# jerry102102102/RL_brain_trainer

Hardware: AMD Instinct MI355X
Metric: env-steps/sec (whole node), Stage-5 Approach->Finisher PPO loops (rollout + update); value = the Approach loop, finisher.value = the Finisher loop (higher is better)
Workload: dtype f32

## Files before the change

### include/kp1_ppo.h

```cpp
#ifndef KP1_PPO_H
#define KP1_PPO_H

#include <stdint.h>

#include "kp1.h"

#ifdef __cplusplus
extern "C" {
#endif

int kp1_gae_scan(int32_t device, const float* rewards, const float* values, const uint8_t* dones, const float* last_values,
                 float gamma, float gae_lambda, float* advantages, float* returns, int32_t T, int32_t N, void* stream);

int kp1_gae_scan_replicas(int32_t device, const float* rewards, const float* values, const uint8_t* dones, const float* last_values,
                          const float* gamma_lambda, int32_t n_per_replica, float* advantages, float* returns, int32_t T, int32_t N, void* stream);

int kp1_bootstrap_truncated(int32_t device, float* rewards, const float* terminal_values, const uint8_t* dones, float gamma,
                            int64_t count, void* stream);

int kp1_adv_minibatch_sums(int32_t device, const float* advantages, const int64_t* idx, int64_t total, int64_t minibatch, double* out_sums,
                           void* stream);
int kp1_random_permutation(int32_t device, int64_t n, const uint32_t* keys, int64_t* out, void* stream);

int kp1_adv_minibatch_stats(int32_t device, const double* sums, int64_t n_minibatches, float* out_stats, void* stream);
// ... 102 lines not shown
                             float* log_prob, float* next_obs, float* reward, uint8_t* done, float* terminal_obs, void* stream);

int kp1_eval_step(kp1_mlp* m, kp1_env* env, float* obs, float* reward, uint8_t* done, const kp1_eval_buffers* buffers, int32_t step,
                  const double* ready_thresholds , int32_t confirm_steps, void* stream);

int kp1_mlp_loss_grad(kp1_mlp* m, const float* obs, int32_t obs_stride, const int64_t* idx, int32_t n, const float* actions,
                      const float* old_log_prob, const float* advantages, const float* returns, float adv_mean, float adv_inv_std,
                      const float* adv_stats_dev, float clip_range, float ent_coef, float vf_coef, float inv_count, float* grad_out,
                      float* stats_out, int32_t grad_is_zero, void* stream);

#define KP1_MLP_OPT_FUSED 1
#define KP1_MLP_OPT_ACTOR_EXTRA_STEPS 2
#define KP1_MLP_OPT_STEP_COUNT 3
#define KP1_MLP_OPT_PROFILE 4
#define KP1_MLP_OPT_BF16X3_WGRAD 5
#define KP1_MLP_PROFILE_SLOTS 4
#define KP1_MLP_PROFILE_TILE 0
#define KP1_MLP_PROFILE_WGRAD 1
#define KP1_MLP_PROFILE_FINALIZE 2
#define KP1_MLP_PROFILE_ADAM 3
int kp1_mlp_set_option(kp1_mlp* m, int32_t option, int32_t value);
int kp1_mlp_profile_read(kp1_mlp* m, float* out_us , int32_t* out_launches );

int kp1_mlp_adam_step(kp1_mlp* m, float* params, float* grad, float* exp_avg, float* exp_avg_sq, float lr, float eps,
                      float max_grad_norm, int32_t step, int32_t flags, void* stream);

int kp1_mlp_anchor_loss_grad(kp1_mlp* m, const float* obs, int32_t obs_stride, const int64_t* idx, int32_t n, const float* teacher_actions,
                             float loss_weight, float* grad_out, float* loss_out, void* stream);

int kp1_mlp_anchor_adam_step(kp1_mlp* m, float* params, float* grad, float* exp_avg, float* exp_avg_sq, float lr, float eps,
                             float max_grad_norm, int32_t step, void* stream);

int kp1_mlp_placement_check(int32_t device, int32_t n_rows, int32_t* out, void* stream);
int kp1_mlp_time_kernels(kp1_mlp* m, const float* obs, int32_t obs_stride, int32_t n, int32_t iters, float* out_ms, double* out_flops,
                         void* stream);

int kp1_set_obs_stride(kp1_env* env, int32_t stride);

#ifdef __cplusplus
}
#endif
#endif
```

### rl_brain_trainer_amd/csrc/kp1_mlp.hip

```cpp
#include <hip/hip_runtime.h>
#include <hip/hip_ext.h>

#include <cmath>
#include <cstddef>
#include <cstdlib>
#include <cstring>
#include <vector>

#include "../../include/kp1_ppo.h"
#include "kp1_device.hpp"
#include "kp1_host.hpp"

using kp1::fail;
using namespace kp1;

typedef float f32x16 __attribute__((ext_vector_type(16)));
typedef float f32x4 __attribute__((ext_vector_type(4)));

namespace {

constexpr int ACT = KP1_MLP_ACT, HEADS = 8;
constexpr float LOG_SQRT_2PI = 0.9189385332046727f;

enum { EPI_BIAS_TANH = 0, EPI_DTANH = 1 };
// ... 818 lines not shown
  } else if (i < L.a_w) {
    r.p = a.hpart + 9 * Hp + (i - L.v_b2);
  } else if (i < L.a_b) {
    const int64_t e = i - L.a_w;
    r.p = a.hpart + (e / H) * Hp + e % H;
  } else if (i < L.c_w) {
    r.p = a.hpart + 10 * Hp + (i - L.a_b);
  } else if (i < L.c_b) {
    r.p = a.hpart + 7 * Hp + (i - L.c_w);
  } else {
    r.p = a.hpart + 10 * Hp + 7;
  }
  return r;
}

__host__ __device__ inline int64_t finalize_wide_count(const ParamLayout& L) { return ACT + 4 * (int64_t)L.H + (L.total - L.a_w); }
__device__ __forceinline__ int64_t finalize_wide_index(const ParamLayout& L, int64_t e) {
  const int H = L.H;
  if (e < ACT) return L.log_std + e;
  e -= ACT;
  if (e < H) return L.p_b1 + e;
  e -= H;
  if (e < H) return L.p_b2 + e;
  e -= H;
  if (e < H) return L.v_b1 + e;
  e -= H;
  if (e < H) return L.v_b2 + e;
  e -= H;
  return L.a_w + e;
}

__host__ __device__ inline int64_t finalize_vec_items(const ParamLayout& L) { return 2 * ((int64_t)L.H * L.H / 4 + (int64_t)L.H * L.IN / 4); }

template <bool POP = false>
__global__ void __launch_bounds__(256) grad_finalize_kernel(const FinalizeArgs a_, int n_main) {
  const FinalizeArgs a = POP ? finalize_args_replica(a_, blockIdx.y) : a_;
  const ParamLayout& L = a.L;
  __shared__ double sq[4];
  __shared__ float red[8][32];
  float gval = 0.f;
  double gsq = 0.0;
  if ((int)blockIdx.x < n_main) {
    const int64_t j = (int64_t)(blockIdx.x * 256u + threadIdx.x);
    const int64_t per2 = (int64_t)L.H * L.H / 4, per1 = (int64_t)L.H * L.IN / 4;
    if (j < 2 * (per2 + per1)) {
      const float* src;
      int64_t stride, dst;
      int n;
      if (j < 2 * per2) {
        const int net = j >= per2;
        const unsigned rem = (unsigned)(j - net * per2), q4 = (unsigned)(L.H / 4), row = rem / q4, c4 = rem - row * q4;
        src = a.slab2 + net * a.s2_net + (int64_t)row * a.s2_ld + 4 * c4;
        stride = a.s2_chunk; n = a.s2_n;
        dst = (net ? L.v_w2 : L.p_w2) + (int64_t)row * L.H + 4 * c4;
      } else {
        const int64_t k = j - 2 * per2;
        const int net = k >= per1;
        const unsigned rem = (unsigned)(k - net * per1), q4 = (unsigned)(L.IN / 4), row = rem / q4, c4 = rem - row * q4;
        src = a.slab1 + net * a.s1_net + (int64_t)row * a.s1_ld + 4 * c4;
        stride = a.s1_chunk; n = a.s1_n;
        dst = (net ? L.v_w1 : L.p_w1) + (int64_t)row * L.IN + 4 * c4;
      }
      f32x4 s = {0.f, 0.f, 0.f, 0.f};
      int c = 0;
      for (; c + 32 <= n; c += 32) {
        f32x4 v[32];
#pragma unroll
        for (int u = 0; u < 32; ++u) v[u] = *reinterpret_cast<const f32x4*>(src + (int64_t)(c + u) * stride);
#pragma unroll
        for (int u = 0; u < 32; ++u) s += v[u];
      }
      for (; c + 16 <= n; c += 16) {
        f32x4 v[16];
#pragma unroll
        for (int u = 0; u < 16; ++u) v[u] = *reinterpret_cast<const f32x4*>(src + (int64_t)(c + u) * stride);
#pragma unroll
        for (int u = 0; u < 16; ++u) s += v[u];
      }
      for (; c + 8 <= n; c += 8) {
        f32x4 v[8];
#pragma unroll
        for (int u = 0; u < 8; ++u) v[u] = *reinterpret_cast<const f32x4*>(src + (int64_t)(c + u) * stride);
#pragma unroll
        for (int u = 0; u < 8; ++u) s += v[u];
      }
      for (; c < n; ++c) s += *reinterpret_cast<const f32x4*>(src + (int64_t)c * stride);
#pragma unroll
      for (int q = 0; q < 4; ++q) {
        a.grad[dst + q] = s[q];
        gsq += (double)s[q] * (double)s[q];
      }
    }
    if (a.step_counter && blockIdx.x == 0 && threadIdx.x == 0) *a.step_counter += 1;
    if (a.stats && blockIdx.x == 0 && threadIdx.x == 3) {
      float ent = 0.f;
      for (int k = 0; k < ACT; ++k) ent += 0.5f + LOG_SQRT_2PI + a.log_std[k];
      a.stats[2] += ent;
    }
  } else {
    const int64_t n_wide = finalize_wide_count(L);
    const int el = threadIdx.x & 31, strand = threadIdx.x >> 5;
    const int64_t e = (int64_t)(blockIdx.x - n_main) * 32 + el;
    const bool is_grad = e < n_wide, is_stat = !is_grad && e < n_wide + 3;
    PartialSrc s{};
    int64_t flat = 0;
    if (is_grad) {
      flat = finalize_wide_index(L, e);
      s = finalize_source(a, flat);
    } else if (is_stat) {
      s.p = a.hpart + 10 * L.Hp + 15 + (e - n_wide);
      s.stride = a.h_stride; s.n = a.h_n; s.add = 0.f;
    }
    float part = 0.f;
    if (is_grad || is_stat) {
      int c = strand;
      for (; c + 8 * 31 < s.n; c += 8 * 32) {
        float v[32];
#pragma unroll
        for (int u = 0; u < 32; ++u) v[u] = s.p[(int64_t)(c + 8 * u) * s.stride];
#pragma unroll
        for (int u = 0; u < 32; ++u) part += v[u];
      }
      for (; c < s.n; c += 8) part += s.p[(int64_t)c * s.stride];
    }
    red[strand][el] = part;
    __syncthreads();
    if (threadIdx.x < 32) {
      float t = red[0][el];
#pragma unroll
      for (int k = 1; k < 8; ++k) t += red[k][el];
      if (is_grad) {
        gval = t + s.add;
        a.grad[flat] = gval;
      } else if (is_stat && a.stats) {
        const int k = (int)(e - n_wide);
        a.stats[k == 2 ? 3 : k] += t * a.inv_count;
      }
    }
  }
  double w = gsq + (double)gval * (double)gval;
  for (int off = 32; off > 0; off >>= 1) w += __shfl_xor(w, off);
  if ((threadIdx.x & 63) == 0) sq[threadIdx.x >> 6] = w;
  __syncthreads();
  if (threadIdx.x == 0) a.sumsq[blockIdx.x] = ((sq[0] + sq[1]) + sq[2]) + sq[3];
}

template <bool POP = false>
__global__ void __launch_bounds__(256) sumsq_partials_kernel(const float* __restrict__ g, int64_t n, double* __restrict__ partials, unsigned r_partials) {
  __shared__ double s[256];
  if constexpr (POP) {
    g += blockIdx.y * (unsigned)n;
    partials += blockIdx.y * r_partials;
  }
  double a = 0.0;
  for (int64_t i = (int64_t)blockIdx.x * 256 + threadIdx.x; i < n; i += (int64_t)gridDim.x * 256) a += (double)g[i] * (double)g[i];
  s[threadIdx.x] = a;
  __syncthreads();
  for (int k = 128; k > 0; k >>= 1) {
    if (threadIdx.x < k) s[threadIdx.x] += s[threadIdx.x + k];
    __syncthreads();
  }
  if (threadIdx.x == 0) partials[blockIdx.x] = s[0];
}

constexpr int ADAM_BLOCK = 256, VEC = 1;
template <bool POP = false>
__global__ void __launch_bounds__(ADAM_BLOCK) adam_kernel(float* __restrict__ p, float* __restrict__ g, float* __restrict__ m, float* __restrict__ v,
                                                   int64_t n, const double* __restrict__ partials, int n_partials, float lr, float eps, float max_norm,
                                                   float bc1, float bc2_sqrt, const ParamLayout L, const Packed k_, int zero_grad,
                                                   const int* __restrict__ step_counter, int host_step, const int* __restrict__ actor_extra,
                                                   unsigned r_partials, const float* __restrict__ hparams) {
// ... 253 lines not shown
    m[i] = mn; v[i] = vn; p[i] = pn;
    pack_one(i, pn, L, k);
  }
}

__global__ void anchor_count_kernel(int* __restrict__ actor_extra) { *actor_extra += 1; }

#include "kp1_env_step.inc"
#include "kp1_eval_step.inc"
#include "kp1_mlp_tile.inc"
#include "kp1_mlp_fused.inc"

}

struct kp1_mlp {
  int device = 0, H = 0, Hp = 0, max_batch = 0;
  int K = 1;
  ParamLayout L;
  Packed k{};
  float* h1 = nullptr;
  float* h2 = nullptr;
  float* dz2 = nullptr;
  float* dz1 = nullptr;
  float* xf = nullptr;
  int bf16x3 = 0;
  unsigned short* sp_h1 = nullptr; unsigned short* sp_dz2 = nullptr; unsigned short* sp_dz1 = nullptr; unsigned short* sp_xf = nullptr;
  double* partials = nullptr;
  double* anchor_partials = nullptr;
  float* slab = nullptr;
  float* slab1 = nullptr;
  float* bslab = nullptr;
  float* hpart = nullptr;
  int n_finalize_blocks = 0;
  int* step_dev = nullptr;
  float* hparams_dev = nullptr;
  bool hparams_on = false;
  int last_s2_n = 0, last_s1_n = 0;
  int fused = 1;
  const float* last_params = nullptr;
  bool slab_stale = false;
  std::vector<void*> allocs;
  int profile = 0;
  struct ProfPair { hipEvent_t a, b; };
  std::vector<ProfPair> prof[KP1_MLP_PROFILE_SLOTS];
  int prof_used[KP1_MLP_PROFILE_SLOTS] = {0, 0, 0, 0};
};

namespace {
struct ProfSlotInFlight { hipEvent_t a = nullptr, b = nullptr; bool attached = false; };
thread_local ProfSlotInFlight tl_prof;

struct ProfScope {
  kp1_mlp* m; int slot; hipStream_t stream; bool on;
  ProfScope(kp1_mlp* m_, int slot_, hipStream_t s_) : m(m_), slot(slot_), stream(s_), on(m_->profile != 0) {
    if (!on) return;
    auto& v = m->prof[slot];
    if (m->prof_used[slot] >= (int)v.size()) {
      kp1_mlp::ProfPair p{};
      if (hipEventCreate(&p.a) != hipSuccess || hipEventCreate(&p.b) != hipSuccess) { on = false; return; }
      v.push_back(p);
    }
    tl_prof.a = v[m->prof_used[slot]].a;
    tl_prof.b = v[m->prof_used[slot]].b;
    tl_prof.attached = false;
  }
  ~ProfScope() {
    if (!on) return;
    if (!tl_prof.attached) {
      (void)hipEventRecord(tl_prof.a, stream);
      (void)hipEventRecord(tl_prof.b, stream);
    }
    tl_prof = ProfSlotInFlight{};
    m->prof_used[slot] += 1;
  }
};

#define KP1_LAUNCH(kernel, grid, block, bytes, stream, ...)                                                        \
  do {                                                                                                             \
    if (tl_prof.a != nullptr && !tl_prof.attached) {                                                               \
      tl_prof.attached = true;                                                                                     \
      hipExtLaunchKernelGGL(kernel, grid, block, bytes, stream, tl_prof.a, tl_prof.b, 0, __VA_ARGS__);             \
    } else {                                                                                                       \
      hipLaunchKernelGGL(kernel, grid, block, bytes, stream, __VA_ARGS__);                                         \
    }                                                                                                              \
  } while (0)
}

namespace {

constexpr int N_PARTIALS = 128;
constexpr int ANCHOR_PARTIALS = 256;
constexpr int PARTIALS_STRIDE = 2 * N_PARTIALS + 2048;
constexpr int TN_SPLIT2 = 8, TN_SPLIT1 = 16;

int tn_chunk_rows(int n, int tiles) {
  int chunks = (256 + tiles - 1) / tiles;
  if (chunks > 64) chunks = 64;
  if (chunks < 1) chunks = 1;
  int rows = (n + chunks - 1) / chunks;
  rows = (rows + 63) / 64 * 64;
  return rows < 64 ? 64 : rows;
}

int mlp_check_device(const kp1_mlp* m) {
  HIP_TRY(hipSetDevice(m->device));
  return KP1_OK;
}

constexpr size_t TN_LDS_BYTES = sizeof(float) * 2 * 2 * 64 * (128 + 4);

template <int BN, int EPI, int K, bool POP = false>
int launch_nt_inst(const GemmNT& g, hipStream_t stream) {
  constexpr int NTH = BN == 256 ? 512 : 256;
  constexpr int BM = 64;
  constexpr int BKS = 32;
  size_t bytes = sizeof(float) * (BM * (size_t)(K + 4) + 2 * (size_t)BN * (BKS + 4));
  const size_t epi = sizeof(float) * (BM * (size_t)(BN + 4) + (size_t)(NTH / (BN / 4)) * BN);
  if (epi > bytes) bytes = epi;
  HIP_TRY(hipFuncSetAttribute((const void*)gemm_nt_kernel<BN, EPI, K, NTH, BM, BKS, POP>, hipFuncAttributeMaxDynamicSharedMemorySize, (int)bytes));
  hipLaunchKernelGGL((gemm_nt_kernel<BN, EPI, K, NTH, BM, BKS, POP>), dim3((g.M + BM - 1) / BM, g.N / BN, POP ? 2 * g.reps : 2), dim3(NTH), bytes, stream, g);
  return KP1_OK;
}

int nt_row_tiles(int n, int Hp) {
  (void)Hp;
  return (n + 63) / 64;
// ... 51 lines not shown
}

int launch_fused_infer_env(const FusedArgs& fa, int env_mode, hipStream_t stream) {
  const size_t bytes = sizeof(float) * FU_LDS_FLOATS;
  const dim3 grid((fa.n + FU_BM - 1) / FU_BM, 1, fa.value ? 2 : 1);
  if (env_mode == KP1_MODE_DOCK) {
    HIP_TRY(hipFuncSetAttribute((const void*)mlp_tile_kernel<false, 2, 2>, hipFuncAttributeMaxDynamicSharedMemorySize, (int)bytes));
    hipLaunchKernelGGL((mlp_tile_kernel<false, 2, 2>), grid, dim3(FU_NTH), bytes, stream, fa);
  } else {
    HIP_TRY(hipFuncSetAttribute((const void*)mlp_tile_kernel<false, 2, 1>, hipFuncAttributeMaxDynamicSharedMemorySize, (int)bytes));
    hipLaunchKernelGGL((mlp_tile_kernel<false, 2, 1>), grid, dim3(FU_NTH), bytes, stream, fa);
  }
  return KP1_OK;
}

int launch_fused_infer(const FusedArgs& fa, hipStream_t stream) {
  const size_t bytes = sizeof(float) * FU_LDS_FLOATS;
  const bool want_pi = fa.mean || fa.action || fa.clipped || fa.log_prob;
  if (!want_pi && !fa.value) return KP1_OK;
  FusedArgs f = fa;
  const bool both = want_pi && fa.value;
  if (!both) f.net_base = want_pi ? 0 : 1;
  const dim3 grid((fa.n + FU_BM - 1) / FU_BM, 1, both ? 2 : 1);
  if (fa.inp == 64) {
    HIP_TRY(hipFuncSetAttribute((const void*)mlp_tile_kernel<false, 2>, hipFuncAttributeMaxDynamicSharedMemorySize, (int)bytes));
    hipLaunchKernelGGL((mlp_tile_kernel<false, 2>), grid, dim3(FU_NTH), bytes, stream, f);
  } else {
    HIP_TRY(hipFuncSetAttribute((const void*)mlp_tile_kernel<false, 4>, hipFuncAttributeMaxDynamicSharedMemorySize, (int)bytes));
    hipLaunchKernelGGL((mlp_tile_kernel<false, 4>), grid, dim3(FU_NTH), bytes, stream, f);
  }
  return KP1_OK;
}

int launch_tn_frag(const TnFragArgs& t, hipStream_t stream) {
  if (t.n_chunks2 > 64 || t.n_chunks1 > 64) return fail(KP1_ERR_INVALID, "too many batch chunks for the partial-gradient slabs");
  const size_t bytes = sizeof(float) * TN_SPLIT_LDS_FLOATS;
  HIP_TRY(hipFuncSetAttribute((const void*)gemm_tn_split_kernel, hipFuncAttributeMaxDynamicSharedMemorySize, (int)bytes));
  KP1_LAUNCH(gemm_tn_split_kernel, dim3(32 * t.n_chunks2 + 16 * t.n_chunks1), dim3(256), bytes, stream, t);
  return KP1_OK;
}

int launch_forward_layers(kp1_mlp* m, const float* obs, int obs_stride, const int64_t* idx, int n, hipStream_t stream) {
  const int Hp = m->Hp, IN = m->L.IN, INP = m->L.INP;
  const int64_t act_stride = (int64_t)m->max_batch * Hp;
  GemmNT g{};
  g.reps = m->K;
  g.r_A = idx ? 0u : (unsigned)(n * obs_stride); g.r_gather = (unsigned)n;
  g.r_W = (unsigned)(2 * Hp * INP); g.r_bias = (unsigned)(2 * Hp); g.r_C = (unsigned)(2 * act_stride);
  g.A = obs; g.lda = obs_stride; g.strideA = 0; g.gather = idx;
  g.W = m->k.w1p; g.strideW = (int64_t)Hp * INP;
  g.bias = m->k.b1; g.strideBias = Hp;
  g.C = m->h1; g.ldc = Hp; g.strideC = act_stride;
  g.aux = nullptr; g.strideAux = 0; g.colsum = nullptr; g.strideColsum = 0;
  g.M = n; g.N = Hp; g.K = INP; g.Kreal = obs_stride >= INP ? INP : IN;
  int rc = launch_nt<EPI_BIAS_TANH>(g, stream);
  if (rc != KP1_OK) return rc;
  g.A = m->h1; g.lda = Hp; g.strideA = act_stride; g.gather = nullptr;
  g.r_A = (unsigned)(2 * act_stride); g.r_W = (unsigned)(2 * Hp * Hp);
  g.W = m->k.w2; g.strideW = (int64_t)Hp * Hp;
  g.bias = m->k.b2;
  g.C = m->h2;
  g.K = Hp; g.Kreal = Hp;
  rc = launch_nt<EPI_BIAS_TANH>(g, stream);
  if (rc != KP1_OK) return rc;
  HIP_TRY(kp1::launch_status());
  return KP1_OK;
}

}

namespace {
// ... 78 lines not shown
  m->H = hidden;
  m->L = make_layout(hidden, obs_dim);
  m->Hp = m->L.Hp;
  m->max_batch = (max_batch + 127) / 128 * 128;
  const int64_t Hp = m->Hp, mb = m->max_batch, INP = m->L.INP, K = m->K;
  auto alloc = [&](void** p, size_t bytes) -> int {
    if (hipMalloc(p, bytes) != hipSuccess) return fail(KP1_ERR_ALLOC, "hipMalloc failed in kp1_mlp_create");
    m->allocs.push_back(*p);
    return hipMemset(*p, 0, bytes) == hipSuccess ? KP1_OK : fail(KP1_ERR_NO_DEVICE, "hipMemset failed");
  };
  int rc = KP1_OK;
#define MLP_ALLOC(ptr, count) if (rc == KP1_OK) rc = alloc((void**)&(ptr), sizeof(*(ptr)) * (size_t)(count))
  MLP_ALLOC(m->k.w1p, K * 2 * Hp * INP);
  MLP_ALLOC(m->k.b1, K * 2 * Hp);
  MLP_ALLOC(m->k.w2, K * 2 * Hp * Hp);
  MLP_ALLOC(m->k.w2t, K * 2 * Hp * Hp);
  MLP_ALLOC(m->k.w1f, K * 2 * Hp * INP);
  MLP_ALLOC(m->k.w2f, K * 2 * Hp * Hp);
  MLP_ALLOC(m->k.w2tf, K * 2 * Hp * Hp);
  MLP_ALLOC(m->k.b2, K * 2 * Hp);
  MLP_ALLOC(m->k.w3, K * HEADS * Hp);
  MLP_ALLOC(m->k.b3, K * HEADS);
  MLP_ALLOC(m->k.log_std, K * HEADS);
  MLP_ALLOC(m->h1, K * 2 * mb * Hp);
  MLP_ALLOC(m->h2, K * 2 * mb * Hp);
  MLP_ALLOC(m->dz2, K * 2 * mb * Hp);
  MLP_ALLOC(m->dz1, K * 2 * mb * Hp);
  MLP_ALLOC(m->xf, mb * INP);
  MLP_ALLOC(m->partials, K * PARTIALS_STRIDE);
  if (Hp == 128) MLP_ALLOC(m->anchor_partials, K * ANCHOR_PARTIALS);
  MLP_ALLOC(m->slab, K * 64 * 2 * Hp * Hp);
  MLP_ALLOC(m->slab1, K * 64 * 2 * Hp * INP);
  MLP_ALLOC(m->step_dev, 4);
  if (K > 1) MLP_ALLOC(m->hparams_dev, K * HP_FIELDS);
  MLP_ALLOC(m->bslab, K * (mb / 32) * 2 * Hp);
  MLP_ALLOC(m->hpart, K * (mb / 32) * (10 * Hp + 32));
#undef MLP_ALLOC
  if (rc != KP1_OK) {
    kp1_mlp_destroy(m);
    return rc;
  }
  *out = m;
  return KP1_OK;
}
}

extern "C" {

int kp1_mlp_destroy(kp1_mlp* m) {
  if (!m) return KP1_OK;
  (void)hipSetDevice(m->device);
  (void)hipDeviceSynchronize();
  for (void* p : m->allocs) (void)hipFree(p);
  for (void* p : {(void*)m->sp_h1, (void*)m->sp_dz2, (void*)m->sp_dz1, (void*)m->sp_xf}) (void)hipFree(p);
  for (auto& v : m->prof)
    for (auto& pr : v) {
      (void)hipEventDestroy(pr.a);
      (void)hipEventDestroy(pr.b);
    }
  delete m;
  return KP1_OK;
}

int kp1_mlp_set_option(kp1_mlp* m, int32_t option, int32_t value) {
  if (!m) return fail(KP1_ERR_INVALID, "NULL argument");
  if (option == KP1_MLP_OPT_FUSED) {
// ... 250 lines not shown
    a.hpart = m->hpart; a.hpart_stride = hpart_stride;
    a.r_act = (unsigned)(2 * act_stride); a.r_hpart = (unsigned)hpart_rep; a.r_partials = (unsigned)PARTIALS_STRIDE;
    a.hparams = pop && m->hparams_on ? m->hparams_dev : nullptr;
    {
      const dim3 hgrid((n + HEAD_ROWS - 1) / HEAD_ROWS, m->K);
      const size_t hbytes = sizeof(float) * (HEADS * Hp + HEAD_ROWS * 8 + 84 + 2 * HEAD_ROWS * (Hp + 4));
      if (pop) {
        HIP_TRY(hipFuncSetAttribute((const void*)head_train_kernel<128, true>, hipFuncAttributeMaxDynamicSharedMemorySize, (int)hbytes));
        hipLaunchKernelGGL((head_train_kernel<128, true>), hgrid, dim3(256), hbytes, stream, a);
      } else if (Hp == 256) {
        HIP_TRY(hipFuncSetAttribute((const void*)head_train_kernel<256>, hipFuncAttributeMaxDynamicSharedMemorySize, (int)hbytes));
        hipLaunchKernelGGL(head_train_kernel<256>, hgrid, dim3(256), hbytes, stream, a);
      } else {
        HIP_TRY(hipFuncSetAttribute((const void*)head_train_kernel<128>, hipFuncAttributeMaxDynamicSharedMemorySize, (int)hbytes));
        hipLaunchKernelGGL(head_train_kernel<128>, hgrid, dim3(256), hbytes, stream, a);
      }
    }
    GemmNT g{};
    g.A = m->dz2; g.lda = Hp; g.strideA = act_stride; g.gather = nullptr;
    g.W = m->k.w2t; g.strideW = (int64_t)Hp * Hp;
    g.bias = nullptr; g.strideBias = 0;
    g.C = m->dz1; g.ldc = Hp; g.strideC = act_stride;
    g.aux = m->h1; g.strideAux = act_stride;
    g.colsum = m->bslab; g.strideColsum = Hp;
    g.M = n; g.N = Hp; g.K = Hp; g.Kreal = Hp;
    g.reps = m->K;
    g.r_A = g.r_C = g.r_aux = (unsigned)(2 * act_stride); g.r_W = (unsigned)(2 * Hp * Hp);
    g.r_colsum = (unsigned)((m->max_batch / 32) * 2 * Hp);
    rc = launch_nt<EPI_DTANH>(g, stream);
    if (rc != KP1_OK) return rc;
  }

  int s2_n = 0, s1_n = 0;
  if (fused) {
    TnFragArgs t{};
    t.inp = INP;
    t.dz2 = m->dz2; t.h1 = m->h1; t.dz1 = m->dz1; t.act_stride = act_stride; t.xf = m->xf;
    t.slab2 = m->slab; t.s2_net = (int64_t)Hp * Hp; t.s2_chunk = 2 * t.s2_net;
    t.slab1 = m->slab1; t.s1_net = (int64_t)Hp * INP; t.s1_chunk = 2 * t.s1_net;
    t.groups = (n + FU_BM - 1) / FU_BM * (FU_BM / 8);
    auto up8 = [](int v) { return (v + 7) / 8 * 8; };
    t.cg2 = up8((t.groups + TN_SPLIT2 - 1) / TN_SPLIT2);
    t.cg1 = up8((t.groups + TN_SPLIT1 - 1) / TN_SPLIT1);
    t.n_chunks2 = (t.groups + t.cg2 - 1) / t.cg2;
    t.n_chunks1 = (t.groups + t.cg1 - 1) / t.cg1;
    if (m->bf16x3) {
      TnBf16Args b{};
      b.dz2 = m->sp_dz2; b.h1 = m->sp_h1; b.dz1 = m->sp_dz1; b.plane = (int64_t)2 * m->max_batch * Hp; b.net = (int64_t)m->max_batch * Hp;
      b.xf = m->sp_xf; b.plane_x = (int64_t)m->max_batch * INP; b.inp = INP;
      b.slab2 = t.slab2; b.s2_net = t.s2_net; b.s2_chunk = t.s2_chunk; b.slab1 = t.slab1; b.s1_net = t.s1_net; b.s1_chunk = t.s1_chunk;
      b.frags = t.groups / 2; b.cf2 = t.cg2 / 2; b.cf1 = t.cg1 / 2; b.n_chunks2 = t.n_chunks2; b.n_chunks1 = t.n_chunks1;
      const size_t bytes = sizeof(float) * TN_SPLIT_LDS_FLOATS;
      HIP_TRY(hipFuncSetAttribute((const void*)gemm_tn_bf16x3_kernel, hipFuncAttributeMaxDynamicSharedMemorySize, (int)bytes));
      ProfScope ps(m, KP1_MLP_PROFILE_WGRAD, stream);
      KP1_LAUNCH(gemm_tn_bf16x3_kernel, dim3(32 * b.n_chunks2 + 16 * b.n_chunks1), dim3(256), bytes, stream, b);
    } else {
      ProfScope ps(m, KP1_MLP_PROFILE_WGRAD, stream);
      rc = launch_tn_frag(t, stream);
    }
    if (rc != KP1_OK) return rc;
    s2_n = t.n_chunks2;
    s1_n = t.n_chunks1;
  } else {
    GemmTN t{};
    t.B = n;
    t.chunk = tn_chunk_rows(n, (Hp / 128) * (Hp / 128) * 2);
    t.D = m->dz2; t.ldd = Hp; t.strideD = act_stride;
    t.X = m->h1; t.ldx = Hp; t.strideX = act_stride; t.gatherX = nullptr;
    t.Nload = Hp; t.n_i_tiles = Hp / 128;
    rc = launch_tn(m, t, Hp / 128, Hp, m->slab, &s2_n, stream);
    if (rc != KP1_OK) return rc;
    t.D = m->dz1;
    t.X = obs; t.ldx = obs_stride; t.strideX = 0; t.gatherX = idx;
    t.Nload = obs_stride >= INP ? INP : IN; t.n_i_tiles = 1;
    t.chunk = tn_chunk_rows(n, (Hp / 128) * 2);
    rc = launch_tn(m, t, Hp / 128, INP, m->slab1, &s1_n, stream);
    if (rc != KP1_OK) return rc;
  }
  FinalizeArgs f{};
  f.L = L;
  f.slab2 = m->slab; f.s2_ld = Hp; f.s2_net = (int64_t)Hp * Hp; f.s2_chunk = 2 * f.s2_net; f.s2_n = s2_n;
  f.slab1 = m->slab1; f.s1_ld = INP; f.s1_net = (int64_t)Hp * INP; f.s1_chunk = 2 * f.s1_net; f.s1_n = s1_n;
  f.bslab = m->bslab; f.b_net = Hp; f.b_tile = 2 * Hp; f.b_n = fused ? (n + FU_BM - 1) / FU_BM * (FU_BM / 32) : nt_row_tiles(n, Hp);
  f.hpart = m->hpart; f.h_stride = 10 * Hp + 32; f.h_n = (n + HEAD_ROWS - 1) / HEAD_ROWS;
  f.ent_coef = ent_coef; f.inv_count = inv_count; f.log_std = m->k.log_std;
  f.grad = grad_out; f.stats = stats_out; f.sumsq = m->partials + 2 * N_PARTIALS;
  f.step_counter = m->step_dev;
  f.r_slab2 = (unsigned)(64 * f.s2_chunk); f.r_slab1 = (unsigned)(64 * f.s1_chunk); f.r_bslab = (unsigned)((m->max_batch / 32) * 2 * Hp);
  f.r_hpart = (unsigned)hpart_rep; f.r_sumsq = (unsigned)PARTIALS_STRIDE;
  f.hparams = pop && m->hparams_on ? m->hparams_dev : nullptr;
  const int n_main = (int)((finalize_vec_items(L) + 255) / 256);
  m->n_finalize_blocks = n_main + (int)((finalize_wide_count(L) + 3 + 31) / 32);
  if (m->n_finalize_blocks > 2048) return fail(KP1_ERR_INVALID, "parameter vector too large for the sum-of-squares partial buffer");
  {
    ProfScope ps(m, KP1_MLP_PROFILE_FINALIZE, stream);
    if (pop)
      KP1_LAUNCH(grad_finalize_kernel<true>, dim3(m->n_finalize_blocks, m->K), dim3(256), 0, stream, f, n_main);
    else
      KP1_LAUNCH(grad_finalize_kernel<false>, dim3(m->n_finalize_blocks), dim3(256), 0, stream, f, n_main);
  }
  HIP_TRY(kp1::launch_status());
  return KP1_OK;
}

int kp1_mlp_profile_read(kp1_mlp* m, float* out_us, int32_t* out_launches) {
  if (!m || !out_us || !out_launches) return fail(KP1_ERR_INVALID, "NULL argument to kp1_mlp_profile_read");
  int rc = mlp_check_device(m);
  if (rc != KP1_OK) return rc;
  for (int k = 0; k < KP1_MLP_PROFILE_SLOTS; ++k) {
    double total_ms = 0.0;
    for (int i = 0; i < m->prof_used[k]; ++i) {
      HIP_TRY(hipEventSynchronize(m->prof[k][i].b));
      float ms = 0.f;
      HIP_TRY(hipEventElapsedTime(&ms, m->prof[k][i].a, m->prof[k][i].b));
      total_ms += ms;
    }
    out_launches[k] = m->prof_used[k];
    out_us[k] = m->prof_used[k] > 0 ? (float)(total_ms * 1e3 / m->prof_used[k]) : 0.f;
    m->prof_used[k] = 0;
  }
  return KP1_OK;
}

int kp1_mlp_time_kernels(kp1_mlp* m, const float* obs, int32_t obs_stride, int32_t n, int32_t iters, float* out_ms, double* out_flops,
                         void* stream_) {
  if (!m || !obs || !out_ms || !out_flops || iters <= 0) return fail(KP1_ERR_INVALID, "bad argument to kp1_mlp_time_kernels");
  if (m->K > 1) return fail(KP1_ERR_UNSUPPORTED, "kp1_mlp_time_kernels is not available on population handles");
  if (n <= 0 || n > m->max_batch) return fail(KP1_ERR_INVALID, "n exceeds the workspace max_batch");
  int rc = mlp_check_device(m);
  if (rc != KP1_OK) return rc;
  hipStream_t stream = (hipStream_t)stream_;
  const int Hp = m->Hp, IN = m->L.IN, INP = m->L.INP;
  const int64_t act_stride = (int64_t)m->max_batch * Hp;
  hipEvent_t e0, e1;
  HIP_TRY(hipEventCreate(&e0));
  HIP_TRY(hipEventCreate(&e1));
  rc = launch_forward_layers(m, obs, obs_stride, nullptr, n, stream);
  if (rc != KP1_OK) return rc;
  HIP_TRY(hipMemcpyAsync(m->dz2, m->h2, sizeof(float) * 2 * (size_t)act_stride, hipMemcpyDeviceToDevice, stream));
  auto time_it = [&](int which) -> int {
    HIP_TRY(hipEventRecord(e0, stream));
    for (int it = 0; it < iters; ++it) {
      GemmNT g{};
      g.gather = nullptr; g.ldc = Hp; g.strideC = act_stride; g.M = n; g.N = Hp;
      if (which == 0) {
        g.A = m->h1; g.lda = Hp; g.strideA = act_stride; g.W = m->k.w2; g.strideW = (int64_t)Hp * Hp; g.bias = m->k.b2; g.strideBias = Hp;
        g.C = m->h2; g.K = Hp; g.Kreal = Hp;
        if (launch_nt<EPI_BIAS_TANH>(g, stream) != KP1_OK) return KP1_ERR_NO_DEVICE;
      } else if (which == 1) {
        g.A = m->dz2; g.lda = Hp; g.strideA = act_stride; g.W = m->k.w2t; g.strideW = (int64_t)Hp * Hp; g.C = m->dz1; g.aux = m->h1;
        g.strideAux = act_stride; g.K = Hp; g.Kreal = Hp;
        if (launch_nt<EPI_DTANH>(g, stream) != KP1_OK) return KP1_ERR_NO_DEVICE;
      } else if (which == 2) {
        GemmTN t{};
        t.B = n; t.chunk = tn_chunk_rows(n, (Hp / 128) * (Hp / 128) * 2);
        t.D = m->dz2; t.ldd = Hp; t.strideD = act_stride; t.X = m->h1; t.ldx = Hp; t.strideX = act_stride;
        t.Nload = Hp; t.n_i_tiles = Hp / 128;
        if (launch_tn(m, t, Hp / 128, Hp, m->slab, nullptr, stream) != KP1_OK) return KP1_ERR_NO_DEVICE;
      } else if (which == 3) {
        g.A = obs; g.lda = obs_stride; g.strideA = 0; g.W = m->k.w1p; g.strideW = (int64_t)Hp * INP; g.bias = m->k.b1; g.strideBias = Hp;
        g.C = m->h1; g.K = INP; g.Kreal = obs_stride >= INP ? INP : IN;
        if (launch_nt<EPI_BIAS_TANH>(g, stream) != KP1_OK) return KP1_ERR_NO_DEVICE;
      } else if (which == 4) {
        FusedArgs fa{};
        fa.obs = obs; fa.obs_stride = obs_stride; fa.Kreal = obs_stride >= INP ? INP : IN; fa.inp = INP; fa.idx = nullptr; fa.n = n;
        fa.k = m->k;
        fa.actions = m->h2; fa.old_logp = m->h2 + (int64_t)ACT * n; fa.adv = m->h2 + (int64_t)(ACT + 1) * n; fa.ret = m->h2 + (int64_t)(ACT + 2) * n;
        fa.adv_mode = 3; fa.adv_mean = 0.f; fa.adv_inv_std = 1.f;
        fa.clip_range = 0.2f; fa.vf_coef = 0.5f; fa.inv_count = 1.f / n;
        fa.h1 = m->h1; fa.dz2 = m->dz2; fa.dz1 = m->dz1; fa.act_stride = act_stride; fa.xf = m->xf;
        fa.bslab = m->bslab; fa.hpart = m->hpart; fa.hpart_stride = 10 * Hp + 32;
        if (launch_fused(fa, stream) != KP1_OK) return KP1_ERR_NO_DEVICE;
      } else {
        TnFragArgs t{};
    t.inp = INP;
        t.dz2 = m->dz2; t.h1 = m->h1; t.dz1 = m->dz1; t.act_stride = act_stride; t.xf = m->xf;
        t.slab2 = m->slab; t.s2_net = (int64_t)Hp * Hp; t.s2_chunk = 2 * t.s2_net;
        t.slab1 = m->slab1; t.s1_net = (int64_t)Hp * INP; t.s1_chunk = 2 * t.s1_net;
        t.groups = (n + FU_BM - 1) / FU_BM * (FU_BM / 8);
        t.cg2 = ((t.groups + TN_SPLIT2 - 1) / TN_SPLIT2 + 7) / 8 * 8;
        t.cg1 = ((t.groups + TN_SPLIT1 - 1) / TN_SPLIT1 + 7) / 8 * 8;
        t.n_chunks2 = (t.groups + t.cg2 - 1) / t.cg2;
        t.n_chunks1 = (t.groups + t.cg1 - 1) / t.cg1;
        if (launch_tn_frag(t, stream) != KP1_OK) return KP1_ERR_NO_DEVICE;
      }
    }
    HIP_TRY(hipEventRecord(e1, stream));
    HIP_TRY(hipEventSynchronize(e1));
    float ms = 0.f;
    HIP_TRY(hipEventElapsedTime(&ms, e0, e1));
    out_ms[which] = ms / iters;
    return KP1_OK;
  };
  for (int which : {3, 0, 1, 2}) {
    rc = time_it(which);
    if (rc != KP1_OK) return rc;
  }
  out_ms[4] = out_ms[5] = 0.f;
  out_flops[4] = out_flops[5] = 0.0;
  if (Hp == FU_HP) {
    for (int which : {4, 5}) {
      rc = time_it(which);
      if (rc != KP1_OK) return rc;
    }
  }
  const double M = n, H = Hp;
  out_flops[0] = 2.0 * 2.0 * M * H * H;
  out_flops[1] = 2.0 * 2.0 * M * H * H;
  out_flops[2] = 2.0 * 2.0 * M * H * H;
  out_flops[3] = 2.0 * 2.0 * M * H * INP;
  if (Hp == FU_HP) {
    out_flops[4] = 2.0 * 2.0 * M * (H * (double)INP + 2.0 * H * H);
    out_flops[5] = 2.0 * 2.0 * M * (H * H + H * (double)INP);
  }
  (void)hipEventDestroy(e0);
  (void)hipEventDestroy(e1);
  return KP1_OK;
// ... 228 lines not shown
```

### rl_brain_trainer_amd/csrc/kp1_mlp_fused.inc

```

struct TnFragArgs {
  const float* dz2; const float* h1; const float* dz1; int64_t act_stride;
  const float* xf; int inp;
  float* slab2; int64_t s2_net, s2_chunk;
  float* slab1; int64_t s1_net, s1_chunk;
  int groups, cg2, n_chunks2, cg1, n_chunks1;
};

template <int RA, int CB>
__device__ __forceinline__ void tn_split_tile(const float* __restrict__ Af, int a_ncb, const float* __restrict__ Bf, int b_ncb, int g_begin, int g_end,
                                              float* __restrict__ out, int out_ld, float* lds) {
  constexpr int SG = 4;
  const int tid = threadIdx.x, lane = tid & 63, wave = __builtin_amdgcn_readfirstlane(tid >> 6);
  const int per = (max(g_end - g_begin, 0) + 3) >> 2;
  const int gb = min(g_begin + wave * per, g_end), ge = min(gb + per, g_end);
  const int64_t a_gs = (int64_t)a_ncb * 256, b_gs = (int64_t)b_ncb * 256;
  f32x4 ra[2][SG][RA], rb[2][SG][CB];
  f32x16 acc[RA][CB];
#pragma unroll
  for (int r = 0; r < RA; ++r)
#pragma unroll
    for (int c = 0; c < CB; ++c)
#pragma unroll
      for (int e = 0; e < 16; ++e) acc[r][c][e] = 0.f;
// ... 25 lines not shown
      __builtin_amdgcn_sched_barrier(0);
      KP1_TNS_MFMA(1, g + SG)
      __builtin_amdgcn_sched_barrier(0);
    }
#undef KP1_TNS_LOAD
#undef KP1_TNS_MFMA
  }
  KP1_TR(13)
  constexpr int TO = 32 * RA, TI = 32 * CB, LDP = TI + 8, Q = TI / 4;
  float* mine = lds + wave * (TO * LDP);
#pragma unroll
  for (int r = 0; r < RA; ++r)
#pragma unroll
    for (int c = 0; c < CB; ++c)
#pragma unroll
      for (int e = 0; e < 16; ++e) {
        const int o = r * 32 + (e & 3) + 8 * (e >> 2) + 4 * (lane >> 5);
        mine[o * LDP + c * 32 + (lane & 31)] = acc[r][c][e];
      }
  __syncthreads();
  KP1_TR(14)
#pragma unroll
  for (int j = 0; j < TO * Q / 256; ++j) {
    const int f = tid + 256 * j, o = f / Q, q = f % Q;
    const float* p0 = lds + o * LDP + 4 * q;
    const f32x4 v = ((*reinterpret_cast<const f32x4*>(p0) + *reinterpret_cast<const f32x4*>(p0 + TO * LDP)) +
                     *reinterpret_cast<const f32x4*>(p0 + 2 * TO * LDP)) + *reinterpret_cast<const f32x4*>(p0 + 3 * TO * LDP);
    store16_sc1(out, (int64_t)o * out_ld + 4 * q, v);
  }
  KP1_TR(15)
}
constexpr int TN_SPLIT_LDS_FLOATS = 4 * 64 * (64 + 8);

__global__ void __launch_bounds__(256, 2) gemm_tn_split_kernel(const TnFragArgs a) {
  extern __shared__ float lds[];
  KP1_CLK(1, 0)
  const int n2 = 32 * a.n_chunks2;
  if ((int)blockIdx.x < n2) {
    const int chunk = blockIdx.x % a.n_chunks2, tile = blockIdx.x / a.n_chunks2;
    const int net = tile >> 4, ot = (tile >> 2) & 3, it = tile & 3;
    const int g0 = chunk * a.cg2, g1 = min(g0 + a.cg2, a.groups);
    float* out = a.slab2 + chunk * a.s2_chunk + net * a.s2_net + (int64_t)(ot * 64) * FU_HP + it * 64;
    tn_split_tile<2, 2>(a.dz2 + net * a.act_stride + (ot * 2) * 256, 8, a.h1 + net * a.act_stride + (it * 2) * 256, 8, g0, g1, out, FU_HP, lds);
  } else {
    const int id = blockIdx.x - n2;
    const int chunk = id % a.n_chunks1, tile = id / a.n_chunks1;
    const int net = tile >> 3, ot = tile & 7;
    const int g0 = chunk * a.cg1, g1 = min(g0 + a.cg1, a.groups);
    const int inp = a.inp;
    float* out = a.slab1 + chunk * a.s1_chunk + net * a.s1_net + (int64_t)(ot * 32) * inp;
    if (inp == 64)
      tn_split_tile<1, 2>(a.dz1 + net * a.act_stride + ot * 256, 8, a.xf, 2, g0, g1, out, 64, lds);
    else
      tn_split_tile<1, 3>(a.dz1 + net * a.act_stride + ot * 256, 8, a.xf, 4, g0, g1, out, 128, lds);
  }
  KP1_CLK(1, 1)
}

struct TnBf16Args {
  const unsigned short* dz2; const unsigned short* h1; const unsigned short* dz1; int64_t plane, net;
  const unsigned short* xf; int64_t plane_x; int inp;
  float* slab2; int64_t s2_net, s2_chunk;
  float* slab1; int64_t s1_net, s1_chunk;
  int frags, cf2, n_chunks2, cf1, n_chunks1;
};

__device__ __forceinline__ bf16x8 tnb_load(const unsigned short* __restrict__ base, int64_t off) {
  const __amdgpu_buffer_rsrc_t r = __builtin_amdgcn_make_buffer_rsrc(const_cast<unsigned short*>(base), 0, 0x7fffffff, 0x00020000);
  return __builtin_bit_cast(bf16x8, __builtin_amdgcn_raw_buffer_load_b128(r, (int)(off * 2), 0, AUX_SC1));
}

template <int RA, int CB>
__device__ __forceinline__ void tn_bf16_tile(const unsigned short* __restrict__ Af, int64_t a_plane, int a_ncb, const unsigned short* __restrict__ Bf, int64_t b_plane,
                                             int b_ncb, int f_begin, int f_end, float* __restrict__ out, int out_ld, float* lds) {
  const int tid = threadIdx.x, lane = tid & 63, wave = __builtin_amdgcn_readfirstlane(tid >> 6);
  const int per = (max(f_end - f_begin, 0) + 3) >> 2;
  const int fb = min(f_begin + wave * per, f_end), fe = min(fb + per, f_end);
  const int64_t a_fs = (int64_t)a_ncb * 512, b_fs = (int64_t)b_ncb * 512;
  bf16x8 ra[2][3][RA], rb[2][3][CB];
  f32x16 acc[RA][CB];
#pragma unroll
  for (int r = 0; r < RA; ++r)
#pragma unroll
    for (int c = 0; c < CB; ++c)
#pragma unroll
      for (int e = 0; e < 16; ++e) acc[r][c][e] = 0.f;
  if (fb < fe) {
// ... 81 lines not shown
```

Baseline: 11.41 million.

## Fuse weight-gradient chunk reduction and finalize into the split-K TN GEMM launch

The split-K weight-gradient kernel now uses per-tile atomic tickets so the last-arriving chunk block sums all partial slabs, writes the final gradient and a sum-of-squares partial. The wide (bias/log_std/head) finalize work and the step/entropy stats also move into the layer-1 blocks. This removes the separate grad_finalize launch and one pass re-reading the slabs. The cost is a memset of the tickets when they are dirty, serialized tail work in the last block, and reliance on ticket reset correctness. A debug readback entry point is added.

After: 11.35 million. Within noise of the previous version (-0.5%).

```diff
diff --git a/include/kp1_ppo.h b/include/kp1_ppo.h
--- a/include/kp1_ppo.h
+++ b/include/kp1_ppo.h
@@ -158,6 +158,7 @@
                              float max_grad_norm, int32_t step, void* stream);
 
 int kp1_mlp_placement_check(int32_t device, int32_t n_rows, int32_t* out, void* stream);
+int kp1_mlp_debug_wgrad_state(kp1_mlp* m, uint32_t* out_tickets , double* out_partials, int32_t* out_n_partials, void* stream);
 int kp1_mlp_time_kernels(kp1_mlp* m, const float* obs, int32_t obs_stride, int32_t n, int32_t iters, float* out_ms, double* out_flops,
                          void* stream);
 
diff --git a/rl_brain_trainer_amd/csrc/kp1_mlp.hip b/rl_brain_trainer_amd/csrc/kp1_mlp.hip
--- a/rl_brain_trainer_amd/csrc/kp1_mlp.hip
+++ b/rl_brain_trainer_amd/csrc/kp1_mlp.hip
@@ -874,6 +874,51 @@
 
 __host__ __device__ inline int64_t finalize_vec_items(const ParamLayout& L) { return 2 * ((int64_t)L.H * L.H / 4 + (int64_t)L.H * L.IN / 4); }
 
+__device__ __forceinline__ float finalize_wide_block(const FinalizeArgs& a, int wb, float* red) {
+  const ParamLayout& L = a.L;
+  float gval = 0.f;
+  const int64_t n_wide = finalize_wide_count(L);
+  const int el = threadIdx.x & 31, strand = threadIdx.x >> 5;
+  const int64_t e = (int64_t)wb * 32 + el;
+  const bool is_grad = e < n_wide, is_stat = !is_grad && e < n_wide + 3;
+  PartialSrc s{};
+  int64_t flat = 0;
+  if (is_grad) {
+    flat = finalize_wide_index(L, e);
+    s = finalize_source(a, flat);
+  } else if (is_stat) {
+    s.p = a.hpart + 10 * L.Hp + 15 + (e - n_wide);
+    s.stride = a.h_stride; s.n = a.h_n; s.add = 0.f;
+  }
+  float part = 0.f;
+  if (is_grad || is_stat) {
+    int c = strand;
+    for (; c + 8 * 31 < s.n; c += 8 * 32) {
+      float v[32];
+#pragma unroll
+      for (int u = 0; u < 32; ++u) v[u] = s.p[(int64_t)(c + 8 * u) * s.stride];
+#pragma unroll
+      for (int u = 0; u < 32; ++u) part += v[u];
+    }
+    for (; c < s.n; c += 8) part += s.p[(int64_t)c * s.stride];
+  }
+  red[strand * 32 + el] = part;
+  __syncthreads();
+  if (threadIdx.x < 32) {
+    float t = red[el];
+#pragma unroll
+    for (int k = 1; k < 8; ++k) t += red[k * 32 + el];
+    if (is_grad) {
+      gval = t + s.add;
+      a.grad[flat] = gval;
+    } else if (is_stat && a.stats) {
+      const int k = (int)(e - n_wide);
+      a.stats[k == 2 ? 3 : k] += t * a.inv_count;
+    }
+  }
+  return gval;
+}
+
 template <bool POP = false>
 __global__ void __launch_bounds__(256) grad_finalize_kernel(const FinalizeArgs a_, int n_main) {
   const FinalizeArgs a = POP ? finalize_args_replica(a_, blockIdx.y) : a_;
@@ -940,45 +985,7 @@
       a.stats[2] += ent;
     }
   } else {
-    const int64_t n_wide = finalize_wide_count(L);
-    const int el = threadIdx.x & 31, strand = threadIdx.x >> 5;
-    const int64_t e = (int64_t)(blockIdx.x - n_main) * 32 + el;
-    const bool is_grad = e < n_wide, is_stat = !is_grad && e < n_wide + 3;
-    PartialSrc s{};
-    int64_t flat = 0;
-    if (is_grad) {
-      flat = finalize_wide_index(L, e);
-      s = finalize_source(a, flat);
-    } else if (is_stat) {
-      s.p = a.hpart + 10 * L.Hp + 15 + (e - n_wide);
-      s.stride = a.h_stride; s.n = a.h_n; s.add = 0.f;
-    }
-    float part = 0.f;
-    if (is_grad || is_stat) {
-      int c = strand;
-      for (; c + 8 * 31 < s.n; c += 8 * 32) {
-        float v[32];
-#pragma unroll
-        for (int u = 0; u < 32; ++u) v[u] = s.p[(int64_t)(c + 8 * u) * s.stride];
-#pragma unroll
-        for (int u = 0; u < 32; ++u) part += v[u];
-      }
-      for (; c < s.n; c += 8) part += s.p[(int64_t)c * s.stride];
-    }
-    red[strand][el] = part;
-    __syncthreads();
-    if (threadIdx.x < 32) {
-      float t = red[0][el];
-#pragma unroll
-      for (int k = 1; k < 8; ++k) t += red[k][el];
-      if (is_grad) {
-        gval = t + s.add;
-        a.grad[flat] = gval;
-      } else if (is_stat && a.stats) {
-        const int k = (int)(e - n_wide);
-        a.stats[k == 2 ? 3 : k] += t * a.inv_count;
-      }
-    }
+    gval = finalize_wide_block(a, (int)blockIdx.x - n_main, &red[0][0]);
   }
   double w = gsq + (double)gval * (double)gval;
   for (int off = 32; off > 0; off >>= 1) w += __shfl_xor(w, off);
@@ -1298,6 +1305,8 @@
   float* bslab = nullptr;
   float* hpart = nullptr;
   int n_finalize_blocks = 0;
+  unsigned* tickets = nullptr;
+  bool tickets_dirty = false;
   int* step_dev = nullptr;
   float* hparams_dev = nullptr;
   bool hparams_on = false;
@@ -1358,6 +1367,7 @@
 constexpr int ANCHOR_PARTIALS = 256;
 constexpr int PARTIALS_STRIDE = 2 * N_PARTIALS + 2048;
 constexpr int TN_SPLIT2 = 8, TN_SPLIT1 = 16;
+static_assert(TN_SPLIT2 <= TNR_MAX2 && TN_SPLIT1 <= TNR_MAX1, "the in-launch reducers hold one register set per batch chunk");
 
 int tn_chunk_rows(int n, int tiles) {
   int chunks = (256 + tiles - 1) / tiles;
@@ -1475,11 +1485,12 @@
   return KP1_OK;
 }
 
-int launch_tn_frag(const TnFragArgs& t, hipStream_t stream) {
+int launch_tn_frag(const TnFragArgs& t, const TnReduceArgs& rd, hipStream_t stream) {
   if (t.n_chunks2 > 64 || t.n_chunks1 > 64) return fail(KP1_ERR_INVALID, "too many batch chunks for the partial-gradient slabs");
+  if (rd.tickets && (t.n_chunks2 > TNR_MAX2 || t.n_chunks1 > TNR_MAX1)) return fail(KP1_ERR_INVALID, "too many batch chunks for the in-launch reducers");
   const size_t bytes = sizeof(float) * TN_SPLIT_LDS_FLOATS;
   HIP_TRY(hipFuncSetAttribute((const void*)gemm_tn_split_kernel, hipFuncAttributeMaxDynamicSharedMemorySize, (int)bytes));
-  KP1_LAUNCH(gemm_tn_split_kernel, dim3(32 * t.n_chunks2 + 16 * t.n_chunks1), dim3(256), bytes, stream, t);
+  KP1_LAUNCH(gemm_tn_split_kernel, dim3(32 * t.n_chunks2 + 16 * t.n_chunks1), dim3(256), bytes, stream, t, rd);
   return KP1_OK;
 }
 
@@ -1624,6 +1635,7 @@
   MLP_ALLOC(m->slab, K * 64 * 2 * Hp * Hp);
   MLP_ALLOC(m->slab1, K * 64 * 2 * Hp * INP);
   MLP_ALLOC(m->step_dev, 4);
+  MLP_ALLOC(m->tickets, 64);
   if (K > 1) MLP_ALLOC(m->hparams_dev, K * HP_FIELDS);
   MLP_ALLOC(m->bslab, K * (mb / 32) * 2 * Hp);
   MLP_ALLOC(m->hpart, K * (mb / 32) * (10 * Hp + 32));
@@ -1940,8 +1952,9 @@
   }
 
   int s2_n = 0, s1_n = 0;
+  const bool in_launch_reduce = fused && !m->bf16x3;
+  TnFragArgs t{};
   if (fused) {
-    TnFragArgs t{};
     t.inp = INP;
     t.dz2 = m->dz2; t.h1 = m->h1; t.dz1 = m->dz1; t.act_stride = act_stride; t.xf = m->xf;
     t.slab2 = m->slab; t.s2_net = (int64_t)Hp * Hp; t.s2_chunk = 2 * t.s2_net;
@@ -1962,11 +1975,7 @@
       HIP_TRY(hipFuncSetAttribute((const void*)gemm_tn_bf16x3_kernel, hipFuncAttributeMaxDynamicSharedMemorySize, (int)bytes));
       ProfScope ps(m, KP1_MLP_PROFILE_WGRAD, stream);
       KP1_LAUNCH(gemm_tn_bf16x3_kernel, dim3(32 * b.n_chunks2 + 16 * b.n_chunks1), dim3(256), bytes, stream, b);
-    } else {
-      ProfScope ps(m, KP1_MLP_PROFILE_WGRAD, stream);
-      rc = launch_tn_frag(t, stream);
-    }
-    if (rc != KP1_OK) return rc;
+    }
     s2_n = t.n_chunks2;
     s1_n = t.n_chunks1;
   } else {
@@ -1997,6 +2006,25 @@
   f.r_slab2 = (unsigned)(64 * f.s2_chunk); f.r_slab1 = (unsigned)(64 * f.s1_chunk); f.r_bslab = (unsigned)((m->max_batch / 32) * 2 * Hp);
   f.r_hpart = (unsigned)hpart_rep; f.r_sumsq = (unsigned)PARTIALS_STRIDE;
   f.hparams = pop && m->hparams_on ? m->hparams_dev : nullptr;
+  if (in_launch_reduce) {
+    if (m->tickets_dirty) {
+      HIP_TRY(hipMemsetAsync(m->tickets, 0, sizeof(unsigned) * 64, stream));
+      m->tickets_dirty = false;
+    }
+    TnReduceArgs rd{};
+    rd.f = f;
+    rd.tickets = m->tickets;
+    m->n_finalize_blocks = TNR_TILES + 16 * t.n_chunks1;
+    m->tickets_dirty = true;
+    {
+      ProfScope ps(m, KP1_MLP_PROFILE_WGRAD, stream);
+      rc = launch_tn_frag(t, rd, stream);
+    }
+    if (rc != KP1_OK) return rc;
+    HIP_TRY(kp1::launch_status());
+    m->tickets_dirty = false;
+    return KP1_OK;
+  }
   const int n_main = (int)((finalize_vec_items(L) + 255) / 256);
   m->n_finalize_blocks = n_main + (int)((finalize_wide_count(L) + 3 + 31) / 32);
   if (m->n_finalize_blocks > 2048) return fail(KP1_ERR_INVALID, "parameter vector too large for the sum-of-squares partial buffer");
@@ -2027,6 +2055,17 @@
     out_us[k] = m->prof_used[k] > 0 ? (float)(total_ms * 1e3 / m->prof_used[k]) : 0.f;
     m->prof_used[k] = 0;
   }
+  return KP1_OK;
+}
+
+int kp1_mlp_debug_wgrad_state(kp1_mlp* m, uint32_t* out_tickets, double* out_partials, int32_t* out_n_partials, void* stream_) {
+  if (!m || !out_tickets || !out_partials || !out_n_partials) return fail(KP1_ERR_INVALID, "NULL argument to kp1_mlp_debug_wgrad_state");
+  int rc = mlp_check_device(m);
+  if (rc != KP1_OK) return rc;
+  HIP_TRY(hipStreamSynchronize((hipStream_t)stream_));
+  HIP_TRY(hipMemcpy(out_tickets, m->tickets, sizeof(uint32_t) * TNR_TILES, hipMemcpyDeviceToHost));
+  HIP_TRY(hipMemcpy(out_partials, m->partials + 2 * N_PARTIALS, sizeof(double) * (size_t)m->n_finalize_blocks, hipMemcpyDeviceToHost));
+  *out_n_partials = m->n_finalize_blocks;
   return KP1_OK;
 }
 
@@ -2090,7 +2129,7 @@
         t.cg1 = ((t.groups + TN_SPLIT1 - 1) / TN_SPLIT1 + 7) / 8 * 8;
         t.n_chunks2 = (t.groups + t.cg2 - 1) / t.cg2;
         t.n_chunks1 = (t.groups + t.cg1 - 1) / t.cg1;
-        if (launch_tn_frag(t, stream) != KP1_OK) return KP1_ERR_NO_DEVICE;
+        if (launch_tn_frag(t, TnReduceArgs{}, stream) != KP1_OK) return KP1_ERR_NO_DEVICE;
       }
     }
     HIP_TRY(hipEventRecord(e1, stream));
diff --git a/rl_brain_trainer_amd/csrc/kp1_mlp_fused.inc b/rl_brain_trainer_amd/csrc/kp1_mlp_fused.inc
--- a/rl_brain_trainer_amd/csrc/kp1_mlp_fused.inc
+++ b/rl_brain_trainer_amd/csrc/kp1_mlp_fused.inc
@@ -81,27 +81,127 @@
 }
 constexpr int TN_SPLIT_LDS_FLOATS = 4 * 64 * (64 + 8);
 
-__global__ void __launch_bounds__(256, 2) gemm_tn_split_kernel(const TnFragArgs a) {
+constexpr int TNR_MAX2 = 8, TNR_MAX1 = 16;
+constexpr int TNR_TILES = 32 + 16;
+struct TnReduceArgs {
+  FinalizeArgs f;
+  unsigned* tickets;
+};
+
+__device__ __forceinline__ bool tn_arrive(unsigned* ticket, int n_chunks, float* lds) {
+  asm volatile("s_waitcnt vmcnt(0)" ::: "memory");
+  __syncthreads();
+  unsigned* flag = reinterpret_cast<unsigned*>(lds);
+  if (threadIdx.x == 0) {
+    const unsigned drawn = __hip_atomic_fetch_add(ticket, 1u, __ATOMIC_RELAXED, __HIP_MEMORY_SCOPE_AGENT);
+    const bool last = drawn == (unsigned)(n_chunks - 1);
+    if (last) __hip_atomic_store(ticket, 0u, __ATOMIC_RELAXED, __HIP_MEMORY_SCOPE_AGENT);
+    *flag = last ? 1u : 0u;
+  }
+  __syncthreads();
+  const bool last = *flag != 0u;
+  __builtin_amdgcn_fence(__ATOMIC_ACQUIRE, "wavefront");
+  return last;
+}
+
+template <int TO, int Q, int MAXC, int JB>
+__device__ __forceinline__ double tn_reduce_tile(const float* __restrict__ slab0, int ld, int64_t chunk_stride, int n, float* __restrict__ grad, int grad_ld,
+                                                 int rows, int cols) {
+  constexpr int J = TO * Q / 256;
+  static_assert(J % JB == 0, "items per thread must split into whole batches");
+  const int tid = threadIdx.x, c_last = n - 1;
+  double gsq = 0.0;
+#pragma unroll
+  for (int j0 = 0; j0 < J; j0 += JB) {
+    f32x4 v[JB][MAXC];
+#pragma unroll
+    for (int jj = 0; jj < JB; ++jj) {
+      const int f = tid + 256 * (j0 + jj), o = f / Q, q = f % Q;
+#pragma unroll
+      for (int u = 0; u < MAXC; ++u) v[jj][u] = load16_sc1(slab0, (int64_t)o * ld + 4 * q + min(u, c_last) * chunk_stride);
+    }
+#pragma unroll
+    for (int jj = 0; jj < JB; ++jj) {
+      const int f = tid + 256 * (j0 + jj), o = f / Q, q = f % Q;
+      f32x4 s = {0.f, 0.f, 0.f, 0.f};
+#pragma unroll
+      for (int u = 0; u < MAXC; ++u)
+        if (u < n) s += v[jj][u];
+      if (o < rows && 4 * q < cols) {
+#pragma unroll
+        for (int e = 0; e < 4; ++e) {
+          grad[(int64_t)o * grad_ld + 4 * q + e] = s[e];
+          gsq += (double)s[e] * (double)s[e];
+        }
+      }
+    }
+  }
+  return gsq;
+}
+
+__device__ __forceinline__ void tn_block_sumsq(double w, float* lds, double* __restrict__ out) {
+  double* sq = reinterpret_cast<double*>(lds + 4);
+  for (int off = 32; off > 0; off >>= 1) w += __shfl_xor(w, off);
+  if ((threadIdx.x & 63) == 0) sq[threadIdx.x >> 6] = w;
+  __syncthreads();
+  if (threadIdx.x == 0) *out = ((sq[0] + sq[1]) + sq[2]) + sq[3];
+  __syncthreads();
+}
+
+__global__ void __launch_bounds__(256, 2) gemm_tn_split_kernel(const TnFragArgs a, const TnReduceArgs rd) {
   extern __shared__ float lds[];
   KP1_CLK(1, 0)
   const int n2 = 32 * a.n_chunks2;
+  const FinalizeArgs& f = rd.f;
   if ((int)blockIdx.x < n2) {
     const int chunk = blockIdx.x % a.n_chunks2, tile = blockIdx.x / a.n_chunks2;
     const int net = tile >> 4, ot = (tile >> 2) & 3, it = tile & 3;
     const int g0 = chunk * a.cg2, g1 = min(g0 + a.cg2, a.groups);
-    float* out = a.slab2 + chunk * a.s2_chunk + net * a.s2_net + (int64_t)(ot * 64) * FU_HP + it * 64;
-    tn_split_tile<2, 2>(a.dz2 + net * a.act_stride + (ot * 2) * 256, 8, a.h1 + net * a.act_stride + (it * 2) * 256, 8, g0, g1, out, FU_HP, lds);
+    float* tile0 = a.slab2 + net * a.s2_net + (int64_t)(ot * 64) * FU_HP + it * 64;
+    tn_split_tile<2, 2>(a.dz2 + net * a.act_stride + (ot * 2) * 256, 8, a.h1 + net * a.act_stride + (it * 2) * 256, 8, g0, g1, tile0 + chunk * a.s2_chunk, FU_HP, lds);
+    if (rd.tickets && tn_arrive(rd.tickets + tile, a.n_chunks2, lds)) {
+      const int H = f.L.H;
+      float* g = f.grad + (net ? f.L.v_w2 : f.L.p_w2) + (int64_t)(ot * 64) * H + it * 64;
+      const double w = tn_reduce_tile<64, 16, TNR_MAX2, 4>(tile0, FU_HP, a.s2_chunk, a.n_chunks2, g, H, H - ot * 64, H - it * 64);
+      tn_block_sumsq(w, lds, f.sumsq + tile);
+    }
   } else {
     const int id = blockIdx.x - n2;
     const int chunk = id % a.n_chunks1, tile = id / a.n_chunks1;
     const int net = tile >> 3, ot = tile & 7;
     const int g0 = chunk * a.cg1, g1 = min(g0 + a.cg1, a.groups);
     const int inp = a.inp;
-    float* out = a.slab1 + chunk * a.s1_chunk + net * a.s1_net + (int64_t)(ot * 32) * inp;
+    float* tile0 = a.slab1 + net * a.s1_net + (int64_t)(ot * 32) * inp;
+    float* out = tile0 + chunk * a.s1_chunk;
     if (inp == 64)
       tn_split_tile<1, 2>(a.dz1 + net * a.act_stride + ot * 256, 8, a.xf, 2, g0, g1, out, 64, lds);
     else
       tn_split_tile<1, 3>(a.dz1 + net * a.act_stride + ot * 256, 8, a.xf, 4, g0, g1, out, 128, lds);
+    if (rd.tickets) {
+      if (tn_arrive(rd.tickets + 32 + tile, a.n_chunks1, lds)) {
+        const int H = f.L.H, IN = f.L.IN;
+        float* g = f.grad + (net ? f.L.v_w1 : f.L.p_w1) + (int64_t)(ot * 32) * IN;
+        const double w = inp == 64 ? tn_reduce_tile<32, 16, TNR_MAX1, 1>(tile0, 64, a.s1_chunk, a.n_chunks1, g, IN, H - ot * 32, IN)
+                                   : tn_reduce_tile<32, 24, TNR_MAX1, 1>(tile0, 128, a.s1_chunk, a.n_chunks1, g, IN, H - ot * 32, IN);
+        tn_block_sumsq(w, lds, f.sumsq + 32 + tile);
+      }
+      const int n_wgs = 16 * a.n_chunks1, n_wide_blocks = (int)((finalize_wide_count(f.L) + 3 + 31) / 32);
+      double wsq = 0.0;
+      for (int wb = id; wb < n_wide_blocks; wb += n_wgs) {
+        const float gval = finalize_wide_block(f, wb, lds + 16);
+        wsq += (double)gval * (double)gval;
+        __syncthreads();
+      }
+      tn_block_sumsq(wsq, lds, f.sumsq + TNR_TILES + id);
+      if (id == 0) {
+        if (f.step_counter && threadIdx.x == 0) *f.step_counter += 1;
+        if (f.stats && threadIdx.x == 3) {
+          float ent = 0.f;
+          for (int k = 0; k < ACT; ++k) ent += 0.5f + LOG_SQRT_2PI + f.log_std[k];
+          f.stats[2] += ent;
+        }
+      }
+    }
   }
   KP1_CLK(1, 1)
 }
```
